# mpi4py/mpi4py-fft

Measured on AMD Instinct MI355X. Metric: pfft_3d_c2c_1024cubed_fp64_gflops, higher is better.
Workload: dtype f64; 1 GPU; PFFT 3D c2c 1024^3 complex128 forward+backward per step

## Files before the change

mpi4py-fft_amd/csrc/fft_pow2_body.inc:

```
  static_assert(SPLIT || sizeof(real) == 4, "fp64 exchanges split planes");
  using GEO = Geo<N, R, RADS...>;
  constexpr int NT = GEO::TPC, RL = GEO::RL, RS = GEO::RS, NTL = N / RL, NTS = N / RS;
  constexpr bool WL = GEO::UNIFORM && WaveLocal<N, R, COLS>::value && !(FLAGS & 16384);
  constexpr int WORD = SPLIT ? sizeof(real) : 2 * sizeof(real);
  constexpr int CS = Lds<N, COLS, T, WORD == 4, FirstRadix<RADS...>::value>::CS;
  constexpr int PADSH = pad_shift<N, FirstRadix<RADS...>::value, COLS>();
  constexpr bool HALF = MODE == MODE_R2C_H || MODE == MODE_C2R_H;
  constexpr int IOMODE = HALF ? MODE_C2C : MODE;
  static_assert(!HALF || (!COLS && !BIGTW && !(FLAGS & 32)), "packed-real modes: contiguous axis only");
  static_assert(GEO::UNIFORM || ((MODE == MODE_C2C || HALF) && !BIGTW && !(FLAGS & (32 | 128))), "stages of unequal width: complex passes and packed-real rows on natural layouts (fused truncation / padding included)");
  static_assert(!(FLAGS & (2048 | 4096)) || ((MODE == MODE_C2C || HALF) && !(FLAGS & (16 | 128))), "hand-off buffers: plain complex passes and plain packed-real rows");
  constexpr bool PLAIN = (FLAGS & 8192) != 0;
  constexpr bool BLK_IN = (FLAGS & 32768) != 0, BLK_OUT = (FLAGS & 65536) != 0;
  constexpr bool NO_SIGN = !GEO::UNIFORM && HALF && !(FLAGS & (64 | 128 | 4096));
  constexpr bool DEFER_SIGN = NO_SIGN || (!GEO::UNIFORM && MODE == MODE_C2C && !(FLAGS & (64 | 128 | 4096)) && sizeof(real) == 8 &&
                                          serial_loads_f64(N, COLS, (FLAGS & 16) != 0));
  const auto L_in_tlg = PLAIN ? decltype(d.in_tlg)(0) : d.in_tlg;
  const auto L_out_tlg = PLAIN ? decltype(d.out_tlg)(0) : d.out_tlg;
  const auto L_in_lgp = (PLAIN && !BLK_IN) ? decltype(d.in_lgp)(0) : d.in_lgp;
  const auto L_out_lgp = (PLAIN && !BLK_OUT) ? decltype(d.out_lgp)(0) : d.out_lgp;
  const auto L_in_jump = (PLAIN && !BLK_IN) ? decltype(d.in_jump)(0) : d.in_jump;
  const auto L_out_jump = (PLAIN && !BLK_OUT) ? decltype(d.out_jump)(0) : d.out_jump;
  const auto L_in_ilg = PLAIN ? decltype(d.in_ilg)(0) : d.in_ilg;
  const auto L_out_ilg = PLAIN ? decltype(d.out_ilg)(0) : d.out_ilg;
  const auto L_fl_bw = PLAIN ? decltype(d.fl_bw)(0) : d.fl_bw;
  const auto L_flat = PLAIN ? decltype(d.flat)(0) : d.flat;
  const auto L_inner_ld = PLAIN ? decltype(d.inner_ld)(0) : d.inner_ld;
  const auto L_inner_st = PLAIN ? decltype(d.inner_st)(0) : d.inner_st;
  const auto L_out_pad = (PLAIN && !HALF) ? decltype(d.out_pad)(0) : d.out_pad;
  [[maybe_unused]] const SysBuf sys_in(in), sys_out(out);
  const cx<real> *tw = reinterpret_cast<const cx<real> *>(d.tw);
  const int tid = threadIdx.x;
  const int c = COLS ? (tid % T) : (tid / NT);
  const int t = COLS ? (tid / T) : (tid % NT);
  void *col = smem + (size_t)c * CS * WORD;
  const unsigned batch = (unsigned)d.batch, inner = (unsigned)d.inner, mid = (unsigned)d.mid;
  constexpr bool ROWTILES = COLS && !BIGTW;
  const unsigned flat_cols = mid * inner;
  const unsigned chunks = ROWTILES ? ((L_flat ? flat_cols : inner) + T - 1) / T : 1;
  const unsigned ntiles = ROWTILES ? (L_flat ? batch / flat_cols : batch / inner) * chunks : (batch + T - 1) / T;
  const real sy_in = d.conj_in ? (real)-1 : (real)1;
  const real sx_out = (real)(MODE == MODE_R2C_H ? 0.5 * GFFT_SCALE : GFFT_SCALE);
  const real sy_out = d.conj_out ? -sx_out : sx_out;
  const int64_t t_in = (!COLS && L_in_tlg) ? (int64_t)(t >> L_in_tlg) * d.in_tS + (t & ((1 << L_in_tlg) - 1)) : (int64_t)t * d.in_es;
  const int64_t t_out = (!COLS && L_out_tlg) ? (int64_t)(t >> L_out_tlg) * d.out_tS + (t & ((1 << L_out_tlg) - 1)) : (int64_t)t * d.out_es;
  const int64_t pad_shift_in = (FLAGS & 16) ? (int64_t)(d.n - d.tr_N) * d.in_es : 0;
  const int64_t pad_shift_out = (FLAGS & 16) ? (int64_t)(d.n - d.tr_N) * d.out_es : 0;
  const int64_t q_in = (!COLS && L_in_tlg) ? (int64_t)(NTL >> L_in_tlg) * d.in_tS : (int64_t)NTL * d.in_es;
  const int64_t q_out = (!COLS && L_out_tlg) ? (int64_t)(NTS >> L_out_tlg) * d.out_tS : (int64_t)NTS * d.out_es;

  GFFT_TILE_LOOP {
    GFFT_TILE_INDEX
    if (tile >= ntiles) continue;
    int tl = t;
    asm volatile("" : "+v"(tl));
    bool valid, valid_st;
    unsigned o, m, i;
    if constexpr (ROWTILES) {
      const unsigned row = tile / chunks, j = tile - row * chunks;
      if (L_flat) {
        o = row;
        unsigned J = j * T + c;
        valid = valid_st = J < flat_cols;
        if (!valid) J = 0;
        m = J / inner;
        i = J - m * inner;
      } else {
        i = j * T + c;
        valid = i < (L_inner_ld ? (unsigned)L_inner_ld : inner);
        valid_st = i < (L_inner_st ? (unsigned)L_inner_st : inner);
        if (!(valid || valid_st)) i = 0;
        o = row / mid;
        m = row - o * mid;
      }
    } else {
      const unsigned b = tile * T + c;
      valid = valid_st = b < batch;
      const unsigned bb = valid ? b : 0;
      const unsigned bm = bb / inner;
      i = bb - bm * inner;
      o = bm / mid;
      m = bm - o * mid;
    }
    int64_t in0 = (int64_t)o * d.in_os + (int64_t)m * d.in_ms, out0 = (int64_t)o * d.out_os + (int64_t)m * d.out_ms;
    if constexpr (COLS) {
      if (L_fl_bw && i >= (unsigned)L_fl_bw) in0 = (int64_t)o * d.in_os + d.fl_tail + (int64_t)m * d.fl_tail_ms + (i - (unsigned)L_fl_bw);
      else in0 += L_in_ilg ? (int64_t)(i >> L_in_ilg) * d.in_iS + (i & ((1u << L_in_ilg) - 1)) : (int64_t)i * d.in_is;
      out0 += L_out_ilg ? (int64_t)(i >> L_out_ilg) * d.out_iS + (i & ((1u << L_out_ilg) - 1)) : (int64_t)i * d.out_is;
    } else {
      in0 += (int64_t)i * d.in_is;
      out0 += (int64_t)i * d.out_is;
    }
    [[maybe_unused]] const unsigned row_ub = o * inner + i;
    [[maybe_unused]] const bool ub_group = (FLAGS & 128) != 0 && d.ub_minw >= (NTL > NTS ? NTL : NTS);
    cx<real> v[R];
    const int seg_in = RL >> L_in_lgp, seg_out = RS >> L_out_lgp;
    if constexpr (NTL < NT) valid = valid && t < NTL;
    if constexpr (NTS < NT) valid_st = valid_st && t < NTS;
    if (valid) {
      int64_t idx = in0 + t_in;
      int cnt = 0;
#pragma unroll
      for (int q = 0; q < RL; ++q) {
        if constexpr ((FLAGS & 16) != 0) {
          if constexpr (HALF && (FLAGS & 64) != 0) {
            const int e = tl + q * NTL;
            const bool ok = e < d.tr_n, nyq = d.tr_even && e == d.tr_n - 1;
            if constexpr ((FLAGS & 128) != 0) v[q] = reinterpret_cast<const cx<real> *>(in)[uneven_offset(d, row_ub, o, i, ok ? e : 0)];
            else v[q] = reinterpret_cast<const cx<real> *>(in)[ok ? idx : in0];
            v[q].x *= ok ? (nyq ? (real)0.5 : (real)1) : (real)0;
            v[q].y *= (ok && !nyq) ? (real)1 : (real)0;
          } else if constexpr ((FLAGS & 64) != 0) v[q] = tile_load_pad<real, IOMODE>(d, in, in0, idx, pad_shift_in, tl + q * NTL, sy_in);
          else v[q] = tile_load<real, IOMODE, false>(d, in, in0, idx, tl + q * NTL, DEFER_SIGN ? (real)1 : sy_in);
        } else if constexpr (MODE == MODE_C2R_H && (FLAGS & 128) != 0) {
          v[q] = reinterpret_cast<const cx<real> *>(in)[ub_group ? uneven_offset_group<NTL>(d, row_ub, o, i, tl, q) : uneven_offset(d, row_ub, o, i, tl + q * NTL)];
        } else if constexpr ((FLAGS & 4096) != 0) {
          v[q] = sys_in.template ld<real>(idx);
          if constexpr (!HALF) v[q].y *= sy_in;
        } else {
          v[q] = tile_load<real, IOMODE, (FLAGS & 1) != 0>(d, in, in0, idx, tl + q * NTL, DEFER_SIGN ? (real)1 : sy_in);
        }
        int64_t step = q_in;
        if (++cnt == seg_in) {
          cnt = 0;
          step += L_in_jump;
        }
        idx += step;
      }
    } else {
#pragma unroll
      for (int q = 0; q < R; ++q) v[q] = {0, 0};
    }
// ... 95 lines not shown
        v[q].x *= sx_out;
        v[q].y *= sy_out;
      }
      constexpr int PAD = PADSH;
      const int c2 = COLS ? tid / NT : tid % T, t2 = COLS ? tid % NT : tid / T;
      real *w = reinterpret_cast<real *>(col);
      real *r = reinterpret_cast<real *>(smem + (size_t)c2 * CS * WORD);
      const int wb = pad_slot<PAD>(t), rb = pad_slot<PAD>(t2);
      __syncthreads();
#pragma unroll
      for (int q = 0; q < R; ++q) w[wb + pad_slot<PAD>(q * NT)] = v[q].x;
      __syncthreads();
#pragma unroll
      for (int q = 0; q < R; ++q) v[q].x = r[rb + pad_slot<PAD>(q * NT)];
      __syncthreads();
#pragma unroll
      for (int q = 0; q < R; ++q) w[wb + pad_slot<PAD>(q * NT)] = v[q].y;
      __syncthreads();
#pragma unroll
      for (int q = 0; q < R; ++q) v[q].y = r[rb + pad_slot<PAD>(q * NT)];
      const unsigned b2 = tile * T + c2;
      if (b2 < batch) {
        const unsigned bm2 = b2 / inner, i2 = b2 - bm2 * inner, o2 = bm2 / mid, m2 = bm2 - o2 * mid;
        int64_t idx = (int64_t)o2 * d.out_os + (int64_t)m2 * d.out_ms + (int64_t)i2 * d.out_is +
                      (int64_t)t2 * d.out_es;
#pragma unroll
        for (int q = 0; q < R; ++q) {
          if constexpr ((FLAGS & 2048) != 0) sys_out.template st<real>(idx, v[q]);
          else stc<real, (FLAGS & 2) != 0>(reinterpret_cast<cx<real> *>(out) + idx, v[q]);
          idx += q_out;
        }
      }
      if constexpr (WL) __syncthreads();
    } else if (valid_st) {
      int64_t idx = out0 + t_out;
      int cnt = 0;
#pragma unroll
      for (int q = 0; q < RS; ++q) {
        if constexpr ((FLAGS & 16) != 0) {
          if constexpr (HALF && !(FLAGS & 64)) {
            const int e = tl + q * NTS;
            if (e < d.tr_n) {
              const bool nyq = d.tr_even && e == d.tr_n - 1;
              int64_t at = idx;
              if constexpr ((FLAGS & 128) != 0) at = uneven_offset(d, row_ub, o, i, e);
              reinterpret_cast<cx<real> *>(out)[at] = {v[q].x * (nyq ? 2 * sx_out : sx_out), nyq ? (real)0 : v[q].y * sy_out};
            }
          } else if constexpr (!(FLAGS & 64)) tile_store_trunc<real, IOMODE>(d, out, idx, pad_shift_out, tl + q * NTS, v[q], sx_out, sy_out);
          else tile_store<real, IOMODE, false, false>(d, out, idx, tl + q * NTS, m, v[q], sx_out, sy_out);
        } else if constexpr (MODE == MODE_R2C_H && (FLAGS & 128) != 0) {
          reinterpret_cast<cx<real> *>(out)[ub_group ? uneven_offset_group<NTS>(d, row_ub, o, i, tl, q) : uneven_offset(d, row_ub, o, i, tl + q * NTS)] = {v[q].x * sx_out, v[q].y * sy_out};
        } else if constexpr ((FLAGS & 2048) != 0) {
          sys_out.template st<real>(idx, cx<real>{v[q].x * sx_out, v[q].y * sy_out});
        } else {
          tile_store<real, IOMODE, BIGTW, (FLAGS & 2) != 0>(d, out, idx, tl + q * NTS, m, v[q], sx_out, sy_out);
        }
        int64_t step = q_out;
        if (++cnt == seg_out) {
          cnt = 0;
          step += L_out_jump;
        }
        idx += step;
      }
      if constexpr (MODE == MODE_R2C_H && (FLAGS & 128) != 0 && !(FLAGS & 16)) {
        if (tl == 0)
          reinterpret_cast<cx<real> *>(out)[uneven_offset(d, row_ub, o, i, N)] = {(z0.x - z0.y) * 2 * sx_out, 0};
// ... 10 lines not shown
```

mpi4py-fft_amd/csrc/fft_pow2_f64.hip:

```cpp
#include "fft_pow2_impl.h"

namespace gfft {

#define P64(N, R, T, COLS, MINW, ...) \
  launch_pow2_inst<double, N, R, T, COLS, true, MINW, 0, __VA_ARGS__>(d, in, out, s)
#define P64F(N, R, T, COLS, MINW, FLAGS, ...) \
  launch_pow2_inst<double, N, R, T, COLS, true, MINW, FLAGS, __VA_ARGS__>(d, in, out, s)

bool pow2_supported_f64(int n) { return n >= 16 && n <= 4096 && (n & (n - 1)) == 0; }

hipError_t launch_pow2_f64(const PassDesc &d, bool cols, int variant, const void *in, void *out,
                           hipStream_t s) {
  if (!cols) {
    const bool plain = variant == 0 && d.mode == MODE_C2C && !d.tw_hi && !d.tr_dir && 2.0 * (double)d.batch * d.n * sizeof(double) * 2 >= 268435456.0;
    switch (d.n) {
      case 16: return P64(16, 4, 16, false, 1, 4, 4);
      case 32: return P64(32, 8, 16, false, 1, 8, 4);
      case 64: return P64(64, 8, 8, false, 1, 8, 8);
      case 128: return P64(128, 8, 4, false, 1, 8, 8, 2);
      case 256:
        if (plain) return P64F(256, 8, 8, false, 1, 8 | 3, 8, 8, 4);
        return P64(256, 8, 8, false, 1, 8, 8, 4);
      case 512:
        if (plain) return P64F(512, 32, 16, false, 2, 8 | 3, 32, 16);
// ... 51 lines not shown
      case 1024: return P64(1024, 8, 8, true, 1, 8, 8, 8, 2);
      case 2048: return P64(2048, 8, 4, true, 1, 8, 8, 8, 4);
      case 4096: return P64(4096, 8, 2, true, 1, 8, 8, 8, 8);
    }
  } else {
    const bool odd_rows = !strided_lines_whole(d, 16);
    const bool odd_near = odd_rows && d.in_es < 65536 && d.out_es < 65536;
    switch (d.n) {
      case 16: return P64F(16, 4, 16, true, 1, 8, 4, 4);
      case 32: return P64F(32, 8, 16, true, 1, 8, 8, 4);
      case 64: return P64F(64, 8, 16, true, 1, 8, 8, 8);
      case 128: return P64F(128, 8, 16, true, 1, 8, 8, 8, 2);
      case 256:
        if (variant == 0 && d.inner % 32 == 0 && !odd_rows && 2.0 * (double)d.batch * 256 * 16 >= 268435456.0) return P64F(256, 32, 32, true, 2, 8 | 3, 32, 8);
        switch (variant) {
          default: return P64F(256, 8, 16, true, 1, 8, 8, 8, 4);
          case 21: return P64F(256, 32, 32, true, 2, 8 | 3, 32, 8);
        }
      case 512:
        if (variant == 0 && d.inner % 32 == 0 && !odd_rows && d.in_es < 65536 && d.out_es < 65536) return P64F(512, 32, 32, true, 2, 8 | 3, 32, 16);
        if (variant == 0 && odd_near) return P64F(512, 32, 16, true, 2, 8, 32, 16);
        switch (variant) {
          case 21: return P64F(512, 32, 32, true, 2, 8 | 3, 32, 16);
          default: return P64F(512, 32, 16, true, 2, 8 | 3, 32, 16);
          case 15: return P64F(512, 32, 16, true, 2, 8, 32, 16);
          case 17: return P64F(512, 8, 16, true, 1, 8, 8, 8, 8);
#ifdef GFFT_VARIANTS
          case 1: return P64F(512, 8, 8, true, 1, 8, 8, 8, 8);
#endif
        }
      case 1024:
        if (variant == 0 && odd_near) return P64F(1024, 32, 16, true, 2, 8, 32, 32);
        switch (variant) {
          default: return P64F(1024, 32, 16, true, 2, 8 | 3, 32, 32);
          case 15: return P64F(1024, 32, 16, true, 2, 8, 32, 32);
          case 17: return P64F(1024, 16, 16, true, 4, 8, 16, 16, 4);
#ifdef GFFT_VARIANTS
          case 1: return P64F(1024, 8, 8, true, 1, 8, 8, 8, 8, 2);
          case 2: return P64F(1024, 16, 8, true, 1, 8, 16, 16, 4);
          case 3: return P64F(1024, 16, 8, true, 4, 8, 16, 16, 4);
          case 4: return P64F(1024, 8, 4, true, 1, 8, 8, 8, 8, 2);
          case 5: return P64F(1024, 8, 8, true, 1, 4, 8, 8, 8, 2);
          case 6: return P64F(1024, 8, 8, true, 1, 7, 8, 8, 8, 2);
          case 10: return P64F(1024, 16, 16, true, 4, 4, 16, 16, 4);
          case 12: return P64F(1024, 16, 16, true, 4, 8, 8, 8, 8, 2);
          case 13: return P64F(1024, 16, 16, true, 4, 8 | 2, 16, 16, 4);
          case 14: return P64F(1024, 16, 16, true, 4, 8 | 3, 16, 16, 4);
#endif
        }
      case 2048:
        if (variant == 0 && !odd_rows && d.inner % 8 == 0 && 2.0 * (double)d.batch * 2048 * 16 >= 268435456.0)
          return P64F(2048, 16, 8, true, 4, 8 | 3, 16, 16, 8);
        return P64F(2048, 16, 8, true, 4, 8, 16, 16, 8);
      case 4096: return P64F(4096, 16, 4, true, 4, 8, 16, 16, 16);
    }
  }
  return hipErrorInvalidValue;
}

bool pow2_r2r_supported(int n) { return n >= 64 && n <= 4096 && (n & (n - 1)) == 0; }

hipError_t launch_pow2_r2r_f64(const PassDesc &d, bool cols, const void *in, void *out, hipStream_t s) {
  if (!cols) {
    switch (d.n) {
      case 64: return launch_pow2_one<double, 64, 8, 8, false, true, 1, 0, MODE_R2R, false, 8, 8>(d, in, out, s);
      case 128: return launch_pow2_one<double, 128, 8, 4, false, true, 1, 0, MODE_R2R, false, 8, 8, 2>(d, in, out, s);
      case 256: return launch_pow2_one<double, 256, 8, 8, false, true, 1, 0, MODE_R2R, false, 8, 8, 4>(d, in, out, s);
      case 512: return launch_pow2_one<double, 512, 8, 4, false, true, 1, 0, MODE_R2R, false, 8, 8, 8>(d, in, out, s);
      case 1024: return launch_pow2_one<double, 1024, 16, 4, false, true, 1, 0, MODE_R2R, false, 16, 16, 4>(d, in, out, s);
      case 2048: return launch_pow2_one<double, 2048, 16, 2, false, true, 1, 0, MODE_R2R, false, 16, 16, 8>(d, in, out, s);
      case 4096: return launch_pow2_one<double, 4096, 16, 1, false, true, 1, 0, MODE_R2R, false, 16, 16, 16>(d, in, out, s);
    }
  } else {
    switch (d.n) {
      case 64: return launch_pow2_one<double, 64, 8, 16, true, true, 1, 0, MODE_R2R, false, 8, 8>(d, in, out, s);
      case 128: return launch_pow2_one<double, 128, 8, 16, true, true, 1, 0, MODE_R2R, false, 8, 8, 2>(d, in, out, s);
      case 256: return launch_pow2_one<double, 256, 8, 16, true, true, 1, 0, MODE_R2R, false, 8, 8, 4>(d, in, out, s);
// ... 11 lines not shown
```

mpi4py-fft_amd/csrc/fft_pow2_impl.h:

```cpp
#pragma once
#include "gfft_internal.h"
#include "pass_io.h"

namespace gfft {

template <typename real> struct K {
  static constexpr real SQ = (real)0.70710678118654752440084436210485;
  static constexpr real C1 = (real)0.92387953251128675612818318939679;
  static constexpr real S1 = (real)0.38268343236508977172845998403040;
};

template <typename real, int S> __device__ __forceinline__ void dft2(cx<real> *v) {
  cx<real> a = v[0], b = v[S];
  v[0] = a + b;
  v[S] = a - b;
}

template <typename real> __device__ __forceinline__ void bf4(cx<real> &a0, cx<real> &a1, cx<real> &a2, cx<real> &a3) {
  cx<real> t0 = a0 + a2, t1 = a0 - a2, t2 = a1 + a3, t3 = mul_mi(a1 - a3);
  a0 = t0 + t2;
  a1 = t1 + t3;
  a2 = t0 - t2;
  a3 = t1 - t3;
}
// ... 911 lines not shown
  typedef unsigned u4 __attribute__((ext_vector_type(4)));
  typedef unsigned u2 __attribute__((ext_vector_type(2)));
  template <typename real> __device__ __forceinline__ cx<real> ld(int64_t elem) const {
    if constexpr (sizeof(real) == 8) return __builtin_bit_cast(cx<real>, __builtin_amdgcn_raw_buffer_load_b128(r, (unsigned)elem * 16u, 0, GFFT_HANDOFF_AUX));
    else return __builtin_bit_cast(cx<real>, __builtin_amdgcn_raw_buffer_load_b64(r, (unsigned)elem * 8u, 0, GFFT_HANDOFF_AUX));
  }
  template <typename real> __device__ __forceinline__ void st(int64_t elem, cx<real> v) const {
    if constexpr (sizeof(real) == 8) __builtin_amdgcn_raw_buffer_store_b128(__builtin_bit_cast(u4, v), r, (unsigned)elem * 16u, 0, GFFT_HANDOFF_AUX);
    else __builtin_amdgcn_raw_buffer_store_b64(__builtin_bit_cast(u2, v), r, (unsigned)elem * 8u, 0, GFFT_HANDOFF_AUX);
  }
};

constexpr bool in_lengths(int n, const int *list, int count) {
  for (int i = 0; i < count; ++i)
    if (list[i] == n) return true;
  return false;
}
constexpr bool serial_loads_f64(int n, bool cols, bool trunc) {
  constexpr int rows_plain[] = {112, 140, 280, 450, 540, 750, 900, 980, 1050, 1260, 1400, 1792, 2100, 2240, 2800, 3000, 3584};
  constexpr int rows_trunc[] = {1050, 1260, 1680, 2100};
  constexpr int cols_plain[] = {168, 250, 280, 350, 450, 750, 900, 1050, 1260, 1800, 2160};
  constexpr int cols_trunc[] = {150, 180, 450, 540, 588, 750, 840, 900, 1008, 1050, 1260, 1500, 1800, 2160, 2250, 2700};
  return cols ? (trunc ? in_lengths(n, cols_trunc, sizeof cols_trunc / sizeof(int)) : in_lengths(n, cols_plain, sizeof cols_plain / sizeof(int)))
              : (trunc ? in_lengths(n, rows_trunc, sizeof rows_trunc / sizeof(int)) : in_lengths(n, rows_plain, sizeof rows_plain / sizeof(int)));
}

struct NoHook { __device__ __forceinline__ void operator()() const {} };
template <typename real, int N, int R, int T, bool COLS, bool SPLIT, int FLAGS, int MODE, bool BIGTW, int... RADS, typename HOOK = NoHook>
__device__ __forceinline__ void pow2_body(const PassDesc &d, const void *__restrict__ in, void *__restrict__ out,
                                          unsigned char *smem, unsigned k_first, unsigned k_step, unsigned k_end,
                                          unsigned xcd_base, double scale, HOOK &&after_loads = HOOK()) {
#define GFFT_SCALE scale
#define GFFT_TILE_LOOP for (unsigned k = k_first; k < k_end; k += k_step)
#define GFFT_TILE_INDEX const unsigned tile = xcd_base + k;
#define GFFT_AFTER_LOADS after_loads();
#include "fft_pow2_body.inc"
#undef GFFT_TILE_LOOP
#undef GFFT_TILE_INDEX
#undef GFFT_AFTER_LOADS
#undef GFFT_SCALE
}

template <typename real, int N, int R, int T, bool COLS, bool SPLIT, int MINW, int FLAGS, int MODE, bool BIGTW, int... RADS>
__global__ void __launch_bounds__((T * Geo<N, R, RADS...>::TPC), MINW)
fft_pow2_kernel(PassDesc d, const void *__restrict__ in, void *__restrict__ out) {
  extern __shared__ __attribute__((aligned(16))) unsigned char smem[];
  const unsigned per_xcd = (pow2_ntiles<T, COLS, BIGTW>(d) + 7) / 8;
  const unsigned kstep = d.swizzle ? gridDim.x / 8 : gridDim.x;
#define GFFT_TILE_LOOP for (unsigned k = d.swizzle ? blockIdx.x / 8 : blockIdx.x; k < (d.swizzle ? per_xcd : ntiles); k += kstep)
#define GFFT_TILE_INDEX const unsigned tile = d.swizzle ? (blockIdx.x % 8) * per_xcd + k : k;
#define GFFT_AFTER_LOADS
#define GFFT_SCALE d.scale
#include "fft_pow2_body.inc"
#undef GFFT_TILE_LOOP
#undef GFFT_TILE_INDEX
#undef GFFT_AFTER_LOADS
#undef GFFT_SCALE
}


template <typename real_, int N, int R, int T, bool COLS, bool SPLIT, int FLAGS, int MODE, bool BIGTW, int... RADS>
struct PassCfg {
  typedef real_ real;
  static constexpr int threads = T * Geo<N, R, RADS...>::TPC;
  static constexpr int regs_per_thread = R * 2 * (int)(sizeof(real_) / 4);
  static constexpr size_t lds = (size_t)T * Lds<N, COLS, T, (SPLIT && sizeof(real_) == 4), FirstRadix<RADS...>::value>::CS * (SPLIT ? sizeof(real_) : 2 * sizeof(real_));
  template <typename HOOK>
  static __device__ __forceinline__ void tile(const PassDesc &d, const void *in, void *out, unsigned char *smem, unsigned t,
                                              double scale, HOOK &&hook) {
    pow2_body<real_, N, R, T, COLS, SPLIT, FLAGS, MODE, BIGTW, RADS...>(d, in, out, smem, t, 1u, t + 1u, 0u, scale, hook);
  }
  static unsigned ntiles(const PassDesc &d) { return pow2_ntiles<T, COLS, BIGTW>(d); }
};

__device__ __forceinline__ bool wave_of_thread0() { return __builtin_amdgcn_readfirstlane(threadIdx.x) == 0; }

__device__ __forceinline__ void fused_give_up(const FusedDesc &f) {
  if (atomicAdd(&f.ctr[1], 1u) == 0u) {
    atomicAdd(&f.ctr[0], 0x80000000u);
    if (f.host_flag) {
      __hip_atomic_store(f.host_flag, f.plan_id, __ATOMIC_RELAXED, __HIP_MEMORY_SCOPE_SYSTEM);
      __threadfence_system();
    }
// ... 192 lines not shown
  static_assert(threads >= 64 && threads <= 1024, "workgroup size");
  constexpr size_t lds_x = (sizeof...(RADS) > 1 || (FLAGS & 32) || MODE == MODE_R2C_H || MODE == MODE_C2R_H) ? (size_t)T * Lds<N, COLS, T, (SPLIT && sizeof(real) == 4), FirstRadix<RADS...>::value>::CS * (SPLIT ? sizeof(real) : 2 * sizeof(real)) : 0;
  constexpr size_t lds_f = (FLAGS & 16) ? (size_t)T * 2 * sizeof(real) : 0;
  constexpr size_t lds = lds_x > lds_f ? lds_x : lds_f;
  static_assert(lds <= 160 * 1024, "LDS budget");
  if (d.in_lgp || d.out_lgp) {
    const int lg = d.in_lgp > d.out_lgp ? d.in_lgp : d.out_lgp;
    if (((R >> lg) << lg) != R || MODE != MODE_C2C || BIGTW) return hipErrorInvalidValue;
    if ((FLAGS & 16) && ((FLAGS & 64) ? d.in_lgp : d.out_lgp)) return hipErrorInvalidValue;
  }
  if (!COLS && ((d.in_tlg && (NT & ((1 << d.in_tlg) - 1))) || (d.out_tlg && (NT & ((1 << d.out_tlg) - 1)))))
    return hipErrorInvalidValue;
  auto kern = fft_pow2_kernel<real, N, R, T, COLS, SPLIT, MINW, FLAGS, MODE, BIGTW, RADS...>;
  if constexpr (lds > 64 * 1024) {
    static bool attr_set[kMaxDevices] = {};
    const int dev = current_device();
    if (!attr_set[dev]) {
      hipError_t e = hipFuncSetAttribute(reinterpret_cast<const void *>(kern),
                                         hipFuncAttributeMaxDynamicSharedMemorySize, (int)lds);
      if (e != hipSuccess) return e;
      attr_set[dev] = true;
    }
  }
  const int64_t flat_cols = d.mid * d.inner;
  const int64_t ntiles = (COLS && !BIGTW) ? (d.flat ? (d.batch / flat_cols) * ((flat_cols + T - 1) / T)
                                                    : (d.batch / d.inner) * ((d.inner + T - 1) / T))
                                          : (d.batch + T - 1) / T;
  const int64_t cap = d.grid_cap > 0 ? d.grid_cap : pow2_grid_cap();
  int grid = (int)(ntiles < cap ? ntiles : cap);
  PassDesc dd = d;
  if (dd.swizzle) {
    if (grid >= 64) grid = grid / 8 * 8; else dd.swizzle = 0;
  }
  hipLaunchKernelGGL(kern, dim3(grid), dim3(threads), lds, s, dd, in, out);
  return hipGetLastError();
}

template <typename real, int MODE, int N, int R, int T, bool SPLIT, int... RADS>
hipError_t half_launch_all(const PassDesc &d, const void *in, void *out, hipStream_t s);
#ifdef GFFT_VARIANTS
constexpr bool kFusedPadMix5 = true;
#else
constexpr bool kFusedPadMix5 = false;
#endif
template <typename real, int MODE, int N, int R, int T, bool SPLIT, int... RADS>
hipError_t half_launch(const PassDesc &d, const void *in, void *out, hipStream_t s) {
  static_assert(MODE == MODE_R2C_H || MODE == MODE_C2R_H, "packed-real modes");
  if constexpr (R == 20 && !kFusedPadMix5) {
    if (d.tr_dir) return hipErrorInvalidValue;
    if (d.ub_p > 1) return launch_pow2_one<real, N, R, T, false, SPLIT, 1, 128, MODE, false, RADS...>(d, in, out, s);
    return launch_pow2_one<real, N, R, T, false, SPLIT, 1, 0, MODE, false, RADS...>(d, in, out, s);
  } else {
    return half_launch_all<real, MODE, N, R, T, SPLIT, RADS...>(d, in, out, s);
  }
}
template <typename real, int MODE, int N, int R, int T, bool SPLIT, int... RADS>
hipError_t half_launch_all(const PassDesc &d, const void *in, void *out, hipStream_t s) {
  if (d.ub_p > 1 && d.tr_dir == 0)
    return launch_pow2_one<real, N, R, T, false, SPLIT, 1, 128, MODE, false, RADS...>(d, in, out, s);
  if (d.ub_p > 1) {
    if constexpr (MODE == MODE_R2C_H) {
      if (d.tr_dir == 1) return launch_pow2_one<real, N, R, T, false, SPLIT, 1, 16 | 128, MODE, false, RADS...>(d, in, out, s);
    } else {
      if (d.tr_dir == 2) return launch_pow2_one<real, N, R, T, false, SPLIT, 1, 16 | 64 | 128, MODE, false, RADS...>(d, in, out, s);
    }
    return hipErrorInvalidValue;
// ... 53 lines not shown
```

mpi4py-fft_amd/csrc/gfft_internal.h:

```cpp
#pragma once
#include <hip/hip_runtime.h>
#include <stdint.h>

namespace gfft {

constexpr int kMaxDevices = 64;
inline int current_device() {
  int d = 0;
  if (hipGetDevice(&d) != hipSuccess) { (void)hipGetLastError(); d = 0; }
  return (d < 0 || d >= kMaxDevices) ? 0 : d;
}

template <typename T> struct cx { T x, y; };

template <typename T> __device__ __forceinline__ cx<T> operator+(cx<T> a, cx<T> b) { return {a.x + b.x, a.y + b.y}; }
template <typename T> __device__ __forceinline__ cx<T> operator-(cx<T> a, cx<T> b) { return {a.x - b.x, a.y - b.y}; }
template <typename T> __device__ __forceinline__ cx<T> cmul(cx<T> a, cx<T> b) {
  return {a.x * b.x - a.y * b.y, a.x * b.y + a.y * b.x};
}
template <typename T> __device__ __forceinline__ cx<T> mul_mi(cx<T> a) { return {a.y, -a.x}; }
template <typename T> __device__ __forceinline__ cx<T> cswap(cx<T> a) { return {a.y, a.x}; }

enum PassMode { MODE_C2C = 0, MODE_R2C = 1, MODE_C2R = 2, MODE_R2R = 3, MODE_R2C_H = 4, MODE_C2R_H = 5 };

struct PassDesc {
  int n;
  int mode;
  int conj_in;
  int conj_out;
  int swizzle;
  int tr_dir, tr_n, tr_N, tr_even;
  int tr_lgper;
  int64_t tr_jump;
  int64_t batch;
  int64_t mid, inner;
  int64_t inner_ld, inner_st;
  int flat;
  int grid_cap;
  int out_pad;
  int ub_p;
  int ub_minw;
  int ub_start[9];
  int64_t ub_rows;
  int64_t in_os, in_ms, in_is, in_es;
  int64_t out_os, out_ms, out_is, out_es;
  int in_lgp, out_lgp;
  int64_t in_jump, out_jump;
  int in_tlg, out_tlg;
  int64_t in_tS, out_tS;
  int in_ilg, out_ilg;
  int64_t in_iS, out_iS;
  int64_t fl_bw, fl_tail, fl_tail_ms;
  int ub_tlg;
  int64_t ub_n1;
  int64_t ub_base[8];
  const void *r2r_pre, *r2r_post;
  int r2r_n, r2r_pos0, r2r_idx0;
  double scale;
  const void *tw;
  const void *rtw;
  const void *tw_hi, *tw_lo;
  int64_t big_n;
  int tw_L;
// ... 129 lines not shown
```

mpi4py-fft_amd/csrc/plan.cpp:

```cpp
#include "../../include/gfft.h"
#include "gfft_internal.h"

#include <atomic>
#include <cmath>
#include <cstdio>
#include <cstdlib>
#include <cstring>
#include <map>
#include <tuple>
#include <mutex>
#include <string>
#include <thread>
#include <vector>

using namespace gfft;

namespace {

thread_local std::string g_last_error;

int fail(int code, const std::string &msg) {
  g_last_error = msg;
  return code;
}

int hip_fail(hipError_t e, const char *what) {
  return fail(e == hipErrorNoDevice || e == hipErrorInvalidDevice ? GFFT_ERR_NO_DEVICE : GFFT_ERR_HIP,
              std::string(what) + ": " + hipGetErrorString(e));
}

#define HIP_TRY(expr)                                  \
  do {                                                 \
    hipError_t _e = (expr);                            \
    if (_e != hipSuccess) return hip_fail(_e, #expr);  \
  } while (0)

bool g_device_checked = false;
int check_device() {
  if (g_device_checked) return GFFT_OK;
  int n = 0;
  hipError_t e = hipGetDeviceCount(&n);
  if (e != hipSuccess || n <= 0) {
    (void)hipGetLastError();
    return fail(GFFT_ERR_NO_DEVICE, "no HIP device available (libgfft has no host fallback)");
  }
  g_device_checked = true;
  return GFFT_OK;
}

struct Options {
  int grid_cap = 0;
  int variant_rows = 0;
  int variant_cols = 0;
  int force_generic = 0;
  int xcd_swizzle = -1;
  int profile = 0;
  int fused3 = 1;
  int debug_flat = 0;
  int flat_out = 1;
  int mixv_variant = 0;
  int mixv = 1;
  int wtile = 1;
  int plane2d = 1;
  int fuse2 = 1;
  int fuse2_ring = 0, fuse2_lag = 0;
  int fuse2_kinds = 2046;
  int fuse2_f32 = 1;
  int fuse2_wait_ms = 2000;
  int debug_tile_lg = 0, debug_tile_side = 0, debug_tile_stride = 0;
  int64_t fused3_min_bytes = 32 << 20;
  int debug_tw_index = 1, debug_tw_exp = 0;
  Options() {
    if (const char *s = getenv("GFFT_GRID_CAP")) grid_cap = atoi(s);
    if (const char *s = getenv("GFFT_VARIANT_ROWS")) variant_rows = atoi(s);
    if (const char *s = getenv("GFFT_VARIANT_COLS")) variant_cols = atoi(s);
    if (const char *s = getenv("GFFT_FORCE_GENERIC")) force_generic = atoi(s);
    if (const char *s = getenv("GFFT_FUSED3")) fused3 = atoi(s);
    if (const char *s = getenv("GFFT_XCD_SWIZZLE")) xcd_swizzle = atoi(s);
    if (const char *s = getenv("GFFT_FUSE2")) fuse2 = atoi(s);
    if (const char *s = getenv("GFFT_FUSE2_RING")) fuse2_ring = atoi(s);
    if (const char *s = getenv("GFFT_FUSE2_LAG")) fuse2_lag = atoi(s);
    if (const char *s = getenv("GFFT_FUSE2_KINDS")) fuse2_kinds = atoi(s);
    if (const char *s = getenv("GFFT_FUSE2_WAIT_MS")) fuse2_wait_ms = atoi(s);
  }
};
Options &opts() {
  static Options o;
  return o;
// ... 209 lines not shown
          synced = it->first.dev;
        }
        (void)hipFree(it->second.p);
        it = bufs.erase(it);
      } else {
        ++it;
      }
    }
    if (synced >= 0 && synced != here && hipSetDevice(here) != hipSuccess) (void)hipGetLastError();
    if (everything) {
      if (hipDeviceSynchronize() != hipSuccess) (void)hipGetLastError();
      for (void *p : retired) (void)hipFree(p);
      retired.clear();
    }
    return GFFT_OK;
  }
};
ScratchPool &scratch_pool() {
  static ScratchPool p;
  return p;
}
std::atomic<int> g_live_plans{0};

}

struct gfft_plan_s {
  int ndims = 0, kind = 0, precision = 0;
  std::vector<int64_t> sizes_in, sizes_out;
  std::vector<int> axes;
  std::vector<Pass> passes;
  size_t region_bytes[BUF_COUNT] = {0, 0, 0, 0, 0, 0, 0};
  double flops = 0, bytes = 0;
  int variant_rows = 0, variant_cols = 0, xcd_swizzle = 0;
  bool fused3 = false;
  int mixv_variant = 0;
  int64_t ws_pitch = 0;
  int ws_tile = 0;
  std::vector<int64_t> trunc;
  std::vector<std::vector<hipEvent_t>> prof;
  std::vector<void *> device_allocs;
  std::vector<Pass> alt;
  unsigned id = 0;
  int device = 0;
  std::atomic<bool> fused_off{false};
  std::atomic<bool> voided{false};
  int async_slot = -1;
  gfft_plan_s();
  ~gfft_plan_s();
};

namespace {
struct AsyncErrors {
  static constexpr int SLOTS = 256;
  std::mutex m;
  unsigned *flag = nullptr;
  gfft_plan_s *owner[SLOTS] = {};
  std::map<unsigned, gfft_plan_s *> live;
  std::vector<unsigned> orphans;
  unsigned next_id = 1;
  unsigned *word() {
    if (!flag) {
      void *p = nullptr;
      if (hipHostMalloc(&p, SLOTS * sizeof(unsigned), hipHostMallocPortable | hipHostMallocMapped) != hipSuccess) { (void)hipGetLastError(); return nullptr; }
      flag = static_cast<unsigned *>(p);
      for (int i = 0; i < SLOTS; ++i) flag[i] = 0;
    }
// ... 942 lines not shown
    };
    Pass f;
    if (!inverse) {
      Pass &p1 = pl->passes[base], &p2 = pl->passes[base + 1];
      if (p1.d.mode == MODE_R2C_H && p2.cols) {
        PassDesc dA = p1.d, dB = p2.d;
        dA.batch = n1; dA.inner = 1; dA.in_os = n2 / 2; dA.in_is = 0; dA.out_os = P; dA.out_is = 0;
        dB.batch = Pu; dB.in_os = 0; dB.out_os = 0; dB.in_es = P;
        if (make_fused2(pl, FUSED_R2C_PLANES, p1, p2, dA, dB, (int)n0, n1 * n2 * prec, w_i0 * esz, n1 * P * esz, &f)) {
          f.bytes2 = alg(p1) + alg(p2);
          pl->passes[base] = f;
          pl->passes.erase(pl->passes.begin() + base + 1);
        }
      }
    } else {
      Pass &p2 = pl->passes[base + 1], &p3 = pl->passes[base + 2];
      if (p3.d.mode == MODE_C2R_H && p2.cols) {
        PassDesc dA = p2.d, dB = p3.d;
        dA.batch = Pu; dA.in_os = 0; dA.out_os = 0; dA.out_es = P;
        dB.batch = n0; dB.inner = 1; dB.in_is = 0; dB.out_is = 0; dB.in_os = P; dB.out_os = n1 * n2 / 2;
        if (make_fused2(pl, FUSED_COLS_C2R, p2, p3, dA, dB, (int)n1, w_i1 * esz, n2 * prec, n0 * P * esz, &f)) {
          f.bytes2 = alg(p2) + alg(p3);
          pl->passes[base + 1] = f;
          pl->passes.erase(pl->passes.begin() + base + 2);
        }
      }
    }
  }
  pl->fused3 = true;
  if (prec == GFFT_F32 && pl->variant_cols == 0) pl->variant_cols = 2;
  if (prec == GFFT_F64 && real && pl->variant_cols == 0) pl->variant_cols = 17;
  if (prec == GFFT_F64 && !real && pl->variant_cols == 0) pl->variant_cols = 16;
  if (pl->xcd_swizzle < 0 && is_pow2(n0) && is_pow2(n1) && is_pow2(n2) && !(real && prec == GFFT_F32)) pl->xcd_swizzle = 1;
  if (opts().grid_cap <= 0)
    for (Pass &p : pl->passes) p.d.grid_cap = real ? 8192 : ((is_pow2(n0) && is_pow2(n1) && is_pow2(n2)) ? 32768 : 16384);
  return GFFT_OK;
}

hipError_t run_pass(const gfft_plan_s *pl, const Pass &p, const PassDesc &d0, const void *in, void *out,
                    double scale, hipStream_t s) {
  if (p.kind == PK_EMBED) return launch_embed(p.pt, pl->precision, in, out, s);
  if (p.kind == PK_MULB) return launch_mulb(p.pt, pl->precision, out, s);
  if (p.kind == PK_EXTRACT) return launch_extract(p.pt, pl->precision, in, out, scale * p.extra_scale, s);
  PassDesc d = d0;
  const int64_t esz_out = ((d.mode == MODE_C2R || d.mode == MODE_R2R) ? 1 : 2) * (int64_t)pl->precision;
  const int64_t esz_in = ((d.mode == MODE_R2C || d.mode == MODE_R2R) ? 1 : 2) * (int64_t)pl->precision;
  (void)esz_in;
  if (!d.grid_cap && p.regk && !p.cols && !pl->fused3 && opts().grid_cap <= 0) d.grid_cap = 16384;
  if (!d.grid_cap && p.regk && p.cols && !pl->fused3 && opts().grid_cap <= 0 && d.mid == 1 && !d.flat && !d.in_lgp &&
      d.in_es >= ((int64_t)1 << 16) && (d.in_es & (d.in_es - 1)) == 0) d.grid_cap = 16384;
  d.swizzle = pl->xcd_swizzle >= 0 ? pl->xcd_swizzle : (p.cols && !d.flat && ((d.out_es * esz_out) % 128 != 0) ? 1 : 0);
  if ((d.mode == MODE_R2C_H || d.mode == MODE_C2R_H) && real_half_supported(d.n))
    return pl->precision == 8 ? launch_real_half_f64(d, pl->variant_rows, in, out, s)
                              : launch_real_half_f32(d, pl->variant_rows, in, out, s);
  if ((d.mode == MODE_R2C_H || d.mode == MODE_C2R_H) && mixv_supported(d.n))
    return pl->precision == 8 ? launch_real_half_mixv_f64(d, in, out, s) : launch_real_half_mixv_f32(d, in, out, s);
  if (d.mode == MODE_R2C_H || d.mode == MODE_C2R_H)
    return pl->precision == 8 ? launch_real_half_mix_f64(d, in, out, s) : launch_real_half_mix_f32(d, in, out, s);
  if (p.regk && d.mode == MODE_R2R && pow2_r2r_supported(d.n))
    return pl->precision == 8 ? launch_pow2_r2r_f64(d, p.cols, in, out, s) : launch_pow2_r2r_f32(d, p.cols, in, out, s);
  if (p.regk && mix3_supported(d.n)) {
    return pl->precision == 8 ? launch_mix3_f64(d, p.cols, in, out, s) : launch_mix3_f32(d, p.cols, in, out, s);
  }
  if (p.regk && mix5_supported(d.n)) {
    return pl->precision == 8 ? launch_mix5_f64(d, p.cols, in, out, s) : launch_mix5_f32(d, p.cols, in, out, s);
  }
  if (p.regk && mixv_supported(d.n)) {
    return pl->precision == 8 ? launch_mixv_f64(d, p.cols, pl->mixv_variant, in, out, s) : launch_mixv_f32(d, p.cols, pl->mixv_variant, in, out, s);
  }
  if (p.regk) {
    const int variant = p.cols ? pl->variant_cols : pl->variant_rows;
    return pl->precision == 8 ? launch_pow2_f64(d, p.cols, variant, in, out, s)
                              : launch_pow2_f32(d, p.cols, variant, in, out, s);
  }
  return launch_generic(d, p.f, pl->precision, in, out, s);
}

}

namespace gfft {
int pow2_grid_cap() { return opts().grid_cap > 0 ? opts().grid_cap : 4096; }
}

static int build_pair2d(gfft_plan_s *pl, const gfft_iodim *cols, int64_t n2, const gfft_iodim *planes, bool inverse, int cols_first,
// ... 211 lines not shown

int gfft_set_option(const char *key, int value) {
  if (!key) return fail(GFFT_ERR_INVALID, "null option name");
  if (!strcmp(key, "grid_cap")) opts().grid_cap = value;
  else if (!strcmp(key, "variant_rows")) opts().variant_rows = value;
  else if (!strcmp(key, "variant_cols")) opts().variant_cols = value;
  else if (!strcmp(key, "force_generic")) opts().force_generic = value;
  else if (!strcmp(key, "copy_nt")) gfft::g_copy_nt = value;
  else if (!strcmp(key, "fused3")) opts().fused3 = value;
  else if (!strcmp(key, "plane2d")) opts().plane2d = value;
  else if (!strcmp(key, "fuse2")) opts().fuse2 = value;
  else if (!strcmp(key, "fuse2_ring")) opts().fuse2_ring = value;
  else if (!strcmp(key, "fuse2_lag")) opts().fuse2_lag = value;
  else if (!strcmp(key, "fuse2_kinds")) opts().fuse2_kinds = value;
  else if (!strcmp(key, "fuse2_wait_ms")) opts().fuse2_wait_ms = value;
  else if (!strcmp(key, "fuse2_f32")) opts().fuse2_f32 = value;
  else if (!strcmp(key, "fuse2_n512")) gfft::g_fuse2_n512 = value;
  else if (!strcmp(key, "c2r_2048")) gfft::g_c2r_2048 = value;
  else if (!strcmp(key, "fuse2_mixv")) gfft::g_fuse2_mixv = value;
  else if (!strcmp(key, "fuse2_mixed")) gfft::g_fuse2_mixed = value;
  else if (!strcmp(key, "fuse2_f32_n512")) gfft::g_fuse2_f32_n512 = value;
  else if (!strcmp(key, "debug_flat")) opts().debug_flat = value;
  else if (!strcmp(key, "flat_out")) opts().flat_out = value;
  else if (!strcmp(key, "wtile")) opts().wtile = value;
  else if (!strcmp(key, "mixv")) opts().mixv = value;
  else if (!strcmp(key, "mixv_variant")) opts().mixv_variant = value;
  else if (!strcmp(key, "debug_tile_lg")) opts().debug_tile_lg = value;
  else if (!strcmp(key, "debug_tile_side")) opts().debug_tile_side = value;
  else if (!strcmp(key, "debug_tile_stride")) opts().debug_tile_stride = value;
  else if (!strcmp(key, "profile")) opts().profile = value;
  else if (!strcmp(key, "debug_tw_index")) opts().debug_tw_index = value;
  else if (!strcmp(key, "debug_tw_exp")) opts().debug_tw_exp = value;
  else if (!strcmp(key, "xcd_swizzle")) opts().xcd_swizzle = value;
  else if (!strcmp(key, "fused3_min_mib")) opts().fused3_min_bytes = (int64_t)value << 20;
  else return fail(GFFT_ERR_INVALID, std::string("unknown option ") + key);
  return GFFT_OK;
}

int gfft_plan_create(gfft_plan *plan, int ndims, const int64_t *sizes_in, const int64_t *sizes_out,
                     int naxes, const int *axes, int kind, int precision) {
  if (!plan || !sizes_in || !sizes_out || !axes) return fail(GFFT_ERR_INVALID, "null argument");
  *plan = nullptr;
  if (ndims < 1 || ndims > 16 || naxes < 1 || naxes > ndims) return fail(GFFT_ERR_INVALID, "bad ndims/naxes");
  if (precision != GFFT_F32 && precision != GFFT_F64) return fail(GFFT_ERR_INVALID, "precision must be 4 or 8");
  if (kind != GFFT_C2C_FORWARD && kind != GFFT_C2C_BACKWARD && kind != GFFT_R2C && kind != GFFT_C2R)
    return fail(GFFT_ERR_UNSUPPORTED, "only c2c / r2c / c2r kinds are implemented (r2r kinds are out of scope)");
  std::vector<int> ax(axes, axes + naxes);
  std::vector<char> seen(ndims, 0);
  for (int &a : ax) {
    if (a < 0) a += ndims;
    if (a < 0 || a >= ndims || seen[a]) return fail(GFFT_ERR_INVALID, "bad or repeated axis");
    seen[a] = 1;
  }
  const int last = ax.back();
  for (int i = 0; i < ndims; ++i) {
    if (sizes_in[i] < 1 || sizes_out[i] < 1) return fail(GFFT_ERR_INVALID, "sizes must be >= 1");
    if (i == last && kind == GFFT_R2C) {
      if (sizes_out[i] != sizes_in[i] / 2 + 1) return fail(GFFT_ERR_INVALID, "r2c: sizes_out[axis] must be n/2+1");
    } else if (i == last && kind == GFFT_C2R) {
      if (sizes_in[i] != sizes_out[i] / 2 + 1) return fail(GFFT_ERR_INVALID, "c2r: sizes_in[axis] must be n/2+1");
    } else if (sizes_in[i] != sizes_out[i]) {
      return fail(GFFT_ERR_INVALID, "sizes_in and sizes_out may differ only along the halved axis");
    }
  }
  int rc = check_device();
  if (rc) return rc;
// ... 995 lines not shown
```

Baseline: 10330 GFLOP/s.

## Add tile-order permutation for strided f64 column passes on 1024-cubed

Measured after the change: 10490 GFLOP/s, median of 6. +1.5%, better.

```diff
diff --git a/mpi4py-fft_amd/csrc/fft_pow2_body.inc b/mpi4py-fft_amd/csrc/fft_pow2_body.inc
--- a/mpi4py-fft_amd/csrc/fft_pow2_body.inc
+++ b/mpi4py-fft_amd/csrc/fft_pow2_body.inc
@@ -12,6 +12,10 @@
   static_assert(!(FLAGS & (2048 | 4096)) || ((MODE == MODE_C2C || HALF) && !(FLAGS & (16 | 128))), "hand-off buffers: plain complex passes and plain packed-real rows");
   constexpr bool PLAIN = (FLAGS & 8192) != 0;
   constexpr bool BLK_IN = (FLAGS & 32768) != 0, BLK_OUT = (FLAGS & 65536) != 0;
+  constexpr bool ORDER = (FLAGS & 131072) != 0;
+  static_assert(!ORDER || (COLS && !BIGTW && GEO::UNIFORM && MODE == MODE_C2C && !(FLAGS & (16 | 32 | 128 | 2048 | 4096)) &&
+                           (NTL & (NTL - 1)) == 0 && RL % 4 == 0 && RL == RS),
+                "row orders: plain strided complex passes");
   constexpr bool NO_SIGN = !GEO::UNIFORM && HALF && !(FLAGS & (64 | 128 | 4096));
   constexpr bool DEFER_SIGN = NO_SIGN || (!GEO::UNIFORM && MODE == MODE_C2C && !(FLAGS & (64 | 128 | 4096)) && sizeof(real) == 8 &&
                                           serial_loads_f64(N, COLS, (FLAGS & 16) != 0));
@@ -53,6 +57,12 @@
     GFFT_TILE_INDEX
     if (tile >= ntiles) continue;
     int tl = t;
+    [[maybe_unused]] int ord_q0 = 0;
+    if constexpr (ORDER) {
+      const unsigned rot = ((unsigned)d.order >> 14) & 3u, ways = ((unsigned)d.order >> 12) & 3u;
+      if (rot) tl = (int)(((unsigned)t + ord_hash * (rot == 1 ? 5u : 4u)) & (unsigned)(NTL - 1));
+      ord_q0 = ways == 2 ? (int)(ord_hash & 3u) : (ways == 1 ? (int)((ord_hash & 1u) * 2u) : 0);
+    }
     asm volatile("" : "+v"(tl));
     bool valid, valid_st;
     unsigned o, m, i;
@@ -97,7 +107,28 @@
     const int seg_in = RL >> L_in_lgp, seg_out = RS >> L_out_lgp;
     if constexpr (NTL < NT) valid = valid && t < NTL;
     if constexpr (NTS < NT) valid_st = valid_st && t < NTS;
-    if (valid) {
+    if constexpr (ORDER) {
+      if (valid) {
+        const int64_t idx0 = in0 + (int64_t)tl * d.in_es;
+        auto issue = [&](auto q0c) {
+          constexpr int Q0 = decltype(q0c)::value;
+#pragma unroll
+          for (int i = 0; i < RL; ++i) {
+            const int q = (i + Q0) % RL;
+            v[q] = tile_load<real, IOMODE, (FLAGS & 1) != 0>(d, in, in0, idx0 + (int64_t)q * q_in, tl + q * NTL, sy_in);
+          }
+        };
+        switch (ord_q0) {
+          default: issue(std::integral_constant<int, 0>()); break;
+          case 1: issue(std::integral_constant<int, RL / 4>()); break;
+          case 2: issue(std::integral_constant<int, RL / 2>()); break;
+          case 3: issue(std::integral_constant<int, 3 * RL / 4>()); break;
+        }
+      } else {
+#pragma unroll
+        for (int q = 0; q < R; ++q) v[q] = {0, 0};
+      }
+    } else if (valid) {
       int64_t idx = in0 + t_in;
       int cnt = 0;
 #pragma unroll
@@ -259,6 +290,24 @@
         }
       }
       if constexpr (WL) __syncthreads();
+    } else if constexpr (ORDER) {
+      if (valid_st) {
+        const int64_t idx0 = out0 + (int64_t)tl * d.out_es;
+        auto issue = [&](auto q0c) {
+          constexpr int Q0 = decltype(q0c)::value;
+#pragma unroll
+          for (int i = 0; i < RS; ++i) {
+            const int q = (i + Q0) % RS;
+            tile_store<real, IOMODE, false, (FLAGS & 2) != 0>(d, out, idx0 + (int64_t)q * q_out, tl + q * NTS, m, v[q], sx_out, sy_out);
+          }
+        };
+        switch (ord_q0) {
+          default: issue(std::integral_constant<int, 0>()); break;
+          case 1: issue(std::integral_constant<int, RS / 4>()); break;
+          case 2: issue(std::integral_constant<int, RS / 2>()); break;
+          case 3: issue(std::integral_constant<int, 3 * RS / 4>()); break;
+        }
+      }
     } else if (valid_st) {
       int64_t idx = out0 + t_out;
       int cnt = 0;
diff --git a/mpi4py-fft_amd/csrc/fft_pow2_f64.hip b/mpi4py-fft_amd/csrc/fft_pow2_f64.hip
--- a/mpi4py-fft_amd/csrc/fft_pow2_f64.hip
+++ b/mpi4py-fft_amd/csrc/fft_pow2_f64.hip
@@ -107,7 +107,9 @@
       case 1024:
         if (variant == 0 && odd_near) return P64F(1024, 32, 16, true, 2, 8, 32, 32);
         switch (variant) {
-          default: return P64F(1024, 32, 16, true, 2, 8 | 3, 32, 32);
+          default:
+            if (d.order) return P64F(1024, 32, 16, true, 2, 8 | 3 | 131072, 32, 32);
+            return P64F(1024, 32, 16, true, 2, 8 | 3, 32, 32);
           case 15: return P64F(1024, 32, 16, true, 2, 8, 32, 32);
           case 17: return P64F(1024, 16, 16, true, 4, 8, 16, 16, 4);
 #ifdef GFFT_VARIANTS
@@ -118,6 +120,7 @@
           case 5: return P64F(1024, 8, 8, true, 1, 4, 8, 8, 8, 2);
           case 6: return P64F(1024, 8, 8, true, 1, 7, 8, 8, 8, 2);
           case 10: return P64F(1024, 16, 16, true, 4, 4, 16, 16, 4);
+          case 11: return P64F(1024, 32, 16, true, 2, 4 | 8 | 3 | 131072, 32, 32);
           case 12: return P64F(1024, 16, 16, true, 4, 8, 8, 8, 8, 2);
           case 13: return P64F(1024, 16, 16, true, 4, 8 | 2, 16, 16, 4);
           case 14: return P64F(1024, 16, 16, true, 4, 8 | 3, 16, 16, 4);
diff --git a/mpi4py-fft_amd/csrc/fft_pow2_impl.h b/mpi4py-fft_amd/csrc/fft_pow2_impl.h
--- a/mpi4py-fft_amd/csrc/fft_pow2_impl.h
+++ b/mpi4py-fft_amd/csrc/fft_pow2_impl.h
@@ -967,7 +967,7 @@
                                           unsigned xcd_base, double scale, HOOK &&after_loads = HOOK()) {
 #define GFFT_SCALE scale
 #define GFFT_TILE_LOOP for (unsigned k = k_first; k < k_end; k += k_step)
-#define GFFT_TILE_INDEX const unsigned tile = xcd_base + k;
+#define GFFT_TILE_INDEX const unsigned tile = xcd_base + k; [[maybe_unused]] const unsigned ord_hash = 0;
 #define GFFT_AFTER_LOADS after_loads();
 #include "fft_pow2_body.inc"
 #undef GFFT_TILE_LOOP
@@ -983,7 +983,23 @@
   const unsigned per_xcd = (pow2_ntiles<T, COLS, BIGTW>(d) + 7) / 8;
   const unsigned kstep = d.swizzle ? gridDim.x / 8 : gridDim.x;
 #define GFFT_TILE_LOOP for (unsigned k = d.swizzle ? blockIdx.x / 8 : blockIdx.x; k < (d.swizzle ? per_xcd : ntiles); k += kstep)
-#define GFFT_TILE_INDEX const unsigned tile = d.swizzle ? (blockIdx.x % 8) * per_xcd + k : k;
+#define GFFT_TILE_INDEX                                                                                              \
+  unsigned tile = d.swizzle ? (blockIdx.x % 8) * per_xcd + k : k;                                                    \
+  [[maybe_unused]] unsigned ord_hash = 0;                                                                            \
+  if constexpr ((FLAGS & 131072) != 0) {                                                                             \
+    if (d.order && d.swizzle) {                                                                                      \
+      const unsigned x = blockIdx.x % 8, il = 1u << (((unsigned)d.order >> 16) & 3u);                                \
+      const unsigned apart = (((unsigned)d.order >> 19) & 127u) ? (((unsigned)d.order >> 19) & 127u) : 37u;          \
+      unsigned kk = k;                                                                                               \
+      if (il > 1) {                                                                                                  \
+        const unsigned g = k % il, r = k / il, j = r % chunks, s = (r / chunks) * il + g;                            \
+        kk = ((s * apart) % (per_xcd / chunks)) * chunks + j;                                                        \
+      }                                                                                                              \
+      kk = (kk + x * ((unsigned)d.order & 4095u)) % per_xcd;                                                         \
+      tile = x * per_xcd + kk;                                                                                       \
+      ord_hash = (((unsigned)d.order >> 18) & 1u) ? x + k : x;                                                       \
+    }                                                                                                                \
+  }
 #define GFFT_AFTER_LOADS
 #define GFFT_SCALE d.scale
 #include "fft_pow2_body.inc"
@@ -1242,6 +1258,16 @@
   if (dd.swizzle) {
     if (grid >= 64) grid = grid / 8 * 8; else dd.swizzle = 0;
   }
+  if constexpr ((FLAGS & 131072) != 0 && COLS && !BIGTW) {
+    const int64_t chunks = (d.inner + T - 1) / T, il = (int64_t)1 << ((d.order >> 16) & 3);
+    const int64_t apart = ((d.order >> 19) & 127) ? ((d.order >> 19) & 127) : 37;
+    int64_t a = ntiles / 8 / chunks, b = apart;
+    while (b) { const int64_t r = a % b; a = b; b = r; }
+    if (!dd.swizzle || d.flat || d.in_lgp || d.out_lgp || ntiles % 8 || (ntiles / 8) % (il * chunks) || (il > 1 && a != 1))
+      dd.order = 0;
+  } else {
+    dd.order = 0;
+  }
   hipLaunchKernelGGL(kern, dim3(grid), dim3(threads), lds, s, dd, in, out);
   return hipGetLastError();
 }
diff --git a/mpi4py-fft_amd/csrc/gfft_internal.h b/mpi4py-fft_amd/csrc/gfft_internal.h
--- a/mpi4py-fft_amd/csrc/gfft_internal.h
+++ b/mpi4py-fft_amd/csrc/gfft_internal.h
@@ -29,6 +29,7 @@
   int conj_in;
   int conj_out;
   int swizzle;
+  int order;
   int tr_dir, tr_n, tr_N, tr_even;
   int tr_lgper;
   int64_t tr_jump;
diff --git a/mpi4py-fft_amd/csrc/plan.cpp b/mpi4py-fft_amd/csrc/plan.cpp
--- a/mpi4py-fft_amd/csrc/plan.cpp
+++ b/mpi4py-fft_amd/csrc/plan.cpp
@@ -54,6 +54,7 @@
   int variant_cols = 0;
   int force_generic = 0;
   int xcd_swizzle = -1;
+  int tile_order = -1;
   int profile = 0;
   int fused3 = 1;
   int debug_flat = 0;
@@ -329,6 +330,7 @@
   size_t region_bytes[BUF_COUNT] = {0, 0, 0, 0, 0, 0, 0};
   double flops = 0, bytes = 0;
   int variant_rows = 0, variant_cols = 0, xcd_swizzle = 0;
+  int tile_order = -1;
   bool fused3 = false;
   int mixv_variant = 0;
   int64_t ws_pitch = 0;
@@ -1337,6 +1339,8 @@
   if (prec == GFFT_F64 && real && pl->variant_cols == 0) pl->variant_cols = 17;
   if (prec == GFFT_F64 && !real && pl->variant_cols == 0) pl->variant_cols = 16;
   if (pl->xcd_swizzle < 0 && is_pow2(n0) && is_pow2(n1) && is_pow2(n2) && !(real && prec == GFFT_F32)) pl->xcd_swizzle = 1;
+  if (prec == GFFT_F64 && !real && !tr && is_pow2(n0) && is_pow2(n1) && is_pow2(n2))
+    pl->tile_order = (n0 == 1024 && n1 == 1024 && n2 == 1024) ? ((1 << 16) | (3 << 19)) : 0;
   if (opts().grid_cap <= 0)
     for (Pass &p : pl->passes) p.d.grid_cap = real ? 8192 : ((is_pow2(n0) && is_pow2(n1) && is_pow2(n2)) ? 32768 : 16384);
   return GFFT_OK;
@@ -1355,6 +1359,7 @@
   if (!d.grid_cap && p.regk && p.cols && !pl->fused3 && opts().grid_cap <= 0 && d.mid == 1 && !d.flat && !d.in_lgp &&
       d.in_es >= ((int64_t)1 << 16) && (d.in_es & (d.in_es - 1)) == 0) d.grid_cap = 16384;
   d.swizzle = pl->xcd_swizzle >= 0 ? pl->xcd_swizzle : (p.cols && !d.flat && ((d.out_es * esz_out) % 128 != 0) ? 1 : 0);
+  d.order = (pl->tile_order >= 0 && p.regk && p.cols && d.swizzle) ? (opts().tile_order >= 0 ? opts().tile_order : pl->tile_order) : 0;
   if ((d.mode == MODE_R2C_H || d.mode == MODE_C2R_H) && real_half_supported(d.n))
     return pl->precision == 8 ? launch_real_half_f64(d, pl->variant_rows, in, out, s)
                               : launch_real_half_f32(d, pl->variant_rows, in, out, s);
@@ -1632,6 +1637,7 @@
   else if (!strcmp(key, "debug_tw_index")) opts().debug_tw_index = value;
   else if (!strcmp(key, "debug_tw_exp")) opts().debug_tw_exp = value;
   else if (!strcmp(key, "xcd_swizzle")) opts().xcd_swizzle = value;
+  else if (!strcmp(key, "tile_order")) opts().tile_order = value;
   else if (!strcmp(key, "fused3_min_mib")) opts().fused3_min_bytes = (int64_t)value << 20;
   else return fail(GFFT_ERR_INVALID, std::string("unknown option ") + key);
   return GFFT_OK;
```
